# CV-Project2025/Project-NeRF

Measured on NVIDIA B200. Metric: train_rays_per_s, higher is better.
Workload: dtype f16

## Files before the change

### include/b2nerf.h

```cpp
#ifndef B2NERF_H_
#define B2NERF_H_

#include <stddef.h>
#include <stdint.h>

#ifdef __cplusplus
extern "C" {
#endif

#define B2N_ABI_VERSION 14

#define B2N_OK 0
#define B2N_EINVAL (-1)
#define B2N_ECUDA (-2)

typedef void* b2n_stream_t;

int b2n_abi_version(void);
const char* b2n_last_error(void);

int b2n_set_active_rows(const int* rows_device);

enum { B2N_ACT_NONE = 0, B2N_ACT_RELU = 1, B2N_ACT_SIGMOID = 2 };


int b2n_occ_pack_bits(const uint8_t* binary, int64_t n_voxels, uint32_t* bits, b2n_stream_t stream);

int b2n_occ_active_mask(const float* pts, int64_t P, const uint32_t* bits, int R, float offset, float scale,
                        uint8_t* mask, b2n_stream_t stream);

int b2n_occ_update(const float* cur_sigma, float* grid, int64_t n_voxels, int dynamic, float decay, float threshold,
                   uint8_t* binary, uint32_t* bits, int64_t* n_active, b2n_stream_t stream);

int b2n_march_mask(const float* rays_o, const float* rays_d, const float* z_base, const float* z_lo,
                   const float* z_hi, const float* u, const uint32_t* bits, int R, float offset, float scale,
                   int64_t B, int N, float* z, uint32_t* mask_words, int32_t* ray_count, b2n_stream_t stream);

size_t b2n_march_scan_scratch(int64_t B);
int b2n_march_scan(int32_t* ray_count, uint32_t* mask_words, int W, int64_t B, int32_t* ray_offset,
                   int32_t* total_out, void* scratch, b2n_stream_t stream);

int b2n_march_compact(const float* rays_o, const float* rays_d, const float* times, const float* z,
                      const uint32_t* mask_words, const int32_t* ray_offset, int64_t B, int N,
                      int32_t* sample_idx, float* pts, float* dirs, float* t_out, b2n_stream_t stream);

int b2n_composite_fwd(const float* rgb, const float* sigma, const float* dx, const float* z, const float* rays_d,
                      const float* bg, int bg_per_ray, const uint32_t* mask_words, const int32_t* ray_offset,
                      int64_t B, int N, float* color, float* depth, float* acc, float* mean_dx,
                      b2n_stream_t stream);
int b2n_composite_bwd(const float* rgb, const float* sigma, const float* dx, const float* z, const float* rays_d,
                      const float* bg, int bg_per_ray, const uint32_t* mask_words, const int32_t* ray_offset,
                      int64_t B, int N, const float* g_color, const float* g_depth, const float* g_acc,
                      const float* g_mean_dx, float* g_rgb, float* g_sigma, float* g_dx, b2n_stream_t stream);

int b2n_pe_fwd(const float* x, int64_t P, int D, const float* bands, int L, float* out, int ld_out, int col0,
               b2n_stream_t stream);
int b2n_pe_bwd(const float* x, int64_t P, int D, const float* bands, int L, const float* g_out, int ld_g, int col0,
               float* g_x, int accumulate, b2n_stream_t stream);

#define B2N_MAX_LEVELS 32
typedef struct {
  float scale;
  uint32_t res;
  uint32_t size;
  uint32_t offset;
  uint32_t hashed;
} b2n_hash_level;

int b2n_hash_fwd(const float* x, int64_t P, float bound, const float* table, const b2n_hash_level* levels_host,
                 int L, int F, float* out, int ld_out, int col0, b2n_stream_t stream);
int b2n_hash_bwd(const float* x, int64_t P, float bound, const float* table, const b2n_hash_level* levels_host,
                 int L, int F, const float* g_out, int ld_g, int col0, float* g_table, float* g_x, int accumulate_x,
                 int level_begin, int level_end, b2n_stream_t stream);

int b2n_hash_tri_fwd(const float* x, const float* t, int64_t P, float bound, const float* table_start,
                     const float* table_mid, const float* table_end, const b2n_hash_level* levels_host, int L,
                     float* out, int ld_out, b2n_stream_t stream);
int b2n_hash_tri_bwd(const float* x, const float* t, int64_t P, float bound, const b2n_hash_level* levels_host, int L,
                     const float* g_out, int ld_g, float* g_table_start, float* g_table_mid, float* g_table_end,
                     b2n_stream_t stream);

int b2n_linear_fwd(const float* X, int ldx, const float* W, int ldw, const float* b, float* Y, int ldy, int64_t P,
                   int K, int N, int act, b2n_stream_t stream);
int b2n_linear_dgrad(const float* dY, int lddy, const float* W, int ldw, const float* Xact, int ldxa, int act,
                     float* dX, int lddx, int64_t P, int K, int N, int accumulate, b2n_stream_t stream);
int b2n_linear_wgrad(const float* dY, int lddy, const float* X, int ldx, float* dW, int lddw, float* db, int64_t P,
                     int K, int N, b2n_stream_t stream);
int b2n_act_bwd(float* dY, int lddy, const float* Y, int ldy, int64_t P, int N, int act, b2n_stream_t stream);

int b2n_sigma_head_fwd(const float* h, int ldh, int64_t P, float* sigma, b2n_stream_t stream);
int b2n_sigma_head_bwd(const float* h, int ldh, int64_t P, const float* g_sigma, float* g_h, int ldg,
                       b2n_stream_t stream);

int b2n_instant_mlp_fwd(const float* x_enc, int ldx, int pos_dim, const float* dirs, const float* dir_bands,
                        int L_dir, const float* sigma_params, const float* color_params, int64_t P, float* rgb,
                        float* sigma, float in_pad_value, b2n_stream_t stream);
int b2n_instant_mlp_fwd_tc(const float* x_enc, int ldx, int pos_dim, const float* dirs, const float* dir_bands,
                           int L_dir, const float* sigma_params, const float* color_params, int64_t P, float* rgb,
                           float* sigma, float in_pad_value, int* err_flag, b2n_stream_t stream);
int b2n_instant_mlp_bwd(const float* x_enc, int ldx, int pos_dim, const float* dirs, const float* dir_bands,
                        int L_dir, const float* sigma_params, const float* color_params, int64_t P,
                        const float* g_rgb, const float* g_sigma, float* g_x_enc, int ldg, float* g_sigma_params,
                        float* g_color_params, void* work4, float in_pad_value, b2n_stream_t stream);
int b2n_instant_mlp_bwd_tc(const float* x_enc, int ldx, int pos_dim, const float* dirs, const float* dir_bands,
                           int L_dir, const float* sigma_params, const float* color_params, int64_t P,
                           const float* g_rgb, const float* g_sigma, float* g_x_enc, int ldg, float* g_sigma_params,
// ... 65 lines not shown
```

### project-nerf_b200/b2n/_lib.py

```python
from __future__ import annotations

import ctypes
import os

import torch

_HERE = os.path.dirname(os.path.abspath(__file__))
LIB_PATH = os.path.join(os.path.dirname(_HERE), "lib", "libb2nerf.so")

ABI_VERSION = 14

P, L, I, F = ctypes.c_void_p, ctypes.c_int64, ctypes.c_int, ctypes.c_float

SIGNATURES = {
    "b2n_abi_version": [],
    "b2n_last_error": [],
    "b2n_set_active_rows": [P],
    "b2n_occ_pack_bits": [P, L, P, P],
    "b2n_occ_active_mask": [P, L, P, I, F, F, P, P],
    "b2n_occ_update": [P, P, L, I, F, F, P, P, P, P],
    "b2n_march_mask": [P, P, P, P, P, P, P, I, F, F, L, I, P, P, P, P],
    "b2n_march_scan_scratch": [L],
    "b2n_march_scan": [P, P, I, L, P, P, P, P],
    "b2n_march_compact": [P, P, P, P, P, P, L, I, P, P, P, P, P],
    "b2n_composite_fwd": [P, P, P, P, P, P, I, P, P, L, I, P, P, P, P, P],
    "b2n_composite_bwd": [P, P, P, P, P, P, I, P, P, L, I, P, P, P, P, P, P, P, P],
    "b2n_pe_fwd": [P, L, I, P, I, P, I, I, P],
    "b2n_pe_bwd": [P, L, I, P, I, P, I, I, P, I, P],
    "b2n_hash_fwd": [P, L, F, P, P, I, I, P, I, I, P],
    "b2n_hash_bwd": [P, L, F, P, P, I, I, P, I, I, P, P, I, I, I, P],
    "b2n_hash_tri_fwd": [P, P, L, F, P, P, P, P, I, P, I, P],
    "b2n_hash_tri_bwd": [P, P, L, F, P, I, P, I, P, P, P, P],
    "b2n_linear_fwd": [P, I, P, I, P, P, I, L, I, I, I, P],
    "b2n_linear_dgrad": [P, I, P, I, P, I, I, P, I, L, I, I, I, P],
    "b2n_linear_wgrad": [P, I, P, I, P, I, P, L, I, I, P],
    "b2n_act_bwd": [P, I, P, I, L, I, I, P],
    "b2n_sigma_head_fwd": [P, I, L, P, P],
    "b2n_sigma_head_bwd": [P, I, L, P, P, I, P],
    "b2n_instant_mlp_fwd": [P, I, I, P, P, I, P, P, L, P, P, F, P],
    "b2n_instant_mlp_fwd_tc": [P, I, I, P, P, I, P, P, L, P, P, F, P, P],
    "b2n_instant_mlp_bwd": [P, I, I, P, P, I, P, P, L, P, P, P, I, P, P, P, F, P],
    "b2n_instant_mlp_bwd_tc": [P, I, I, P, P, I, P, P, L, P, P, P, I, P, P, P, F, P, P],
    "b2n_fmlp_in_pad": [I],
    "b2n_fmlp_out_pad": [I],
    "b2n_fmlp_fwd": [P, I, I, P, I, I, I, I, P, P, P, I, I, L, P, I, P, P, P],
    "b2n_fmlp_bwd": [I, I, I, I, P, P, I, I, L, P, I, P, I, P, P, P, P, I, P, I, P, P],
    "b2n_fmlp_wgrad_tc": [P, P, P, P, L, I, I, I, P, P, P, P, P, P, P],
    "b2n_fmlp_wgrad": [I, P, P, P, P, P, P, P, P, P, P, P, L, P, P],
    "b2n_nerf_mlp_wgrad": [P, P, P, I, P, L, P, P, P, P, P, P, P, P],
    "b2n_nerf_mlp_dx": [P, P, P, I, P, I, I, L, P, I, P],
    "b2n_nerf_mlp_head_wgrad": [P, P, P, L, P, P, P, P],
    "b2n_nerf_mlp_packed_bytes": [],
    "b2n_nerf_mlp_pack": [P, P, P, I, I, P, P],
    "b2n_nerf_mlp_fwd": [P, I, P, I, P, P, P, P, P, L, P, P, P, P, P, P],
    "b2n_pad_bf16": [P, L, I, I, P, P],
    "b2n_opt_prepare": [P, I, P, P, P],
    "b2n_opt_adamw": [P, I, P, I, P, P, P, P, P],
    "b2n_sample_rays": [P, P, P, P, P, P, L, I, I, I, F, F, P, P, P, P, P],
    "b2n_nerf_mlp_packed_bwd_bytes": [],
    "b2n_nerf_mlp_pack_bwd": [P, P, P, I, I, P, P],
    "b2n_nerf_mlp_bwd": [P, P, P, P, P, P, P, P, L, P, P, P, P],
}
DEBUG_SIGNATURES = {
    "b2n_debug_mlp256_prof": [P],
    "b2n_debug_mlp256_flags": [ctypes.c_int],
    "b2n_debug_mlp256_set_pair": [ctypes.c_int],
    "b2n_debug_hash_variant": [I, I],
    "b2n_debug_hash_config": [P, P],
    "b2n_debug_instant_bwd_groups": [I],
    "b2n_debug_instant_fwd_slots": [I],
    "b2n_debug_gather_bench": [P, L, I, I, P, P],
    "b2n_debug_red_bench": [P, L, I, I, I, P],
    "b2n_debug_mnmajor_probe": [P, P, P, I, I, I, I, P],
}
_RESTYPES = {"b2n_last_error": ctypes.c_char_p, "b2n_march_scan_scratch": ctypes.c_size_t,
             "b2n_nerf_mlp_packed_bytes": ctypes.c_size_t, "b2n_nerf_mlp_packed_bwd_bytes": ctypes.c_size_t}


class HashLevelC(ctypes.Structure):
    _fields_ = [("scale", ctypes.c_float), ("res", ctypes.c_uint32), ("size", ctypes.c_uint32),
                ("offset", ctypes.c_uint32), ("hashed", ctypes.c_uint32)]


def _load():
    if not os.path.exists(LIB_PATH):
        raise ImportError(
            f"{LIB_PATH} not found: build the CUDA extension first (python project-nerf_b200/build.py). "
            "This package has no CPU fallback.")
    lib = ctypes.CDLL(LIB_PATH)
    for name, argtypes in list(SIGNATURES.items()) + list(DEBUG_SIGNATURES.items()):
        fn = getattr(lib, name)
        fn.argtypes = argtypes
        fn.restype = _RESTYPES.get(name, ctypes.c_int)
    v = lib.b2n_abi_version()
    if v != ABI_VERSION:
        raise ImportError(f"libb2nerf.so ABI {v} != binding ABI {ABI_VERSION}: rebuild")
    return lib


lib = _load()

LAUNCHES = {"count": 0}
_KERNELS_PER_CALL = {"b2n_march_scan": 3, "b2n_linear_wgrad": 2, "b2n_instant_mlp_bwd": 2, "b2n_instant_mlp_bwd_tc": 2, "b2n_fmlp_bwd": 2}


def ptr(t):
    return None if t is None else t.data_ptr()


def stream():
    return torch.cuda.current_stream().cuda_stream


class Profiler:

    def __init__(self):
        self.records = []

    def summary(self):
        out = {}
        for name, nbytes, flops, e0, e1 in self.records:
            d = out.setdefault(name, dict(calls=0, ms=0.0, bytes=0.0, flops=0.0))
            d["calls"] += 1
            d["ms"] += e0.elapsed_time(e1)
            d["bytes"] += nbytes
            d["flops"] += flops
        return out


PROFILER = None


def call(name: str, *args, work=(0.0, 0.0)):
    prof = PROFILER
    if prof is not None:
        e0 = torch.cuda.Event(enable_timing=True)
        e1 = torch.cuda.Event(enable_timing=True)
        e0.record()
    rc = getattr(lib, name)(*args)
    if prof is not None:
        e1.record()
        prof.records.append((name, float(work[0]), float(work[1]), e0, e1))
    _raise_on(name, rc)
    LAUNCHES["count"] += _KERNELS_PER_CALL.get(name, 1)


def _raise_on(name, rc):
    if rc != 0:
        msg = lib.b2n_last_error().decode(errors="replace")
        if rc == -1:
            raise ValueError(f"{name}: {msg}")
        raise RuntimeError(f"{name} failed ({rc}): {msg}")


def hash_config():
    v, m = ctypes.c_int(), ctypes.c_int()
    _raise_on("b2n_debug_hash_config", lib.b2n_debug_hash_config(ctypes.byref(v), ctypes.byref(m)))
    return v.value, m.value


class hash_variant:

    def __init__(self, variant, merge_res):
        self.cfg = (variant, merge_res)

    def __enter__(self):
        self.prev = hash_config()
        _raise_on("b2n_debug_hash_variant", lib.b2n_debug_hash_variant(*self.cfg))
        return self

    def __exit__(self, *exc):
        _raise_on("b2n_debug_hash_variant", lib.b2n_debug_hash_variant(*self.prev))
        return False


# ... 53 lines not shown
```

### project-nerf_b200/b2n/ops.py

```python
from __future__ import annotations

import ctypes
import math
from typing import List, Optional, Sequence

import numpy as np
import torch
from torch.amp import custom_bwd, custom_fwd

from . import _lib
from ._lib import HashLevelC, current_rows, ptr, require_cuda, stream, with_ctx_rows

import os as _os
INSTANT_FWD_TC = _os.environ.get("B2N_INSTANT_TC", "1") != "0"
INSTANT_BWD_TC = _os.environ.get("B2N_INSTANT_BWD_TC", "1") != "0"


def call(name, *args, work=(0.0, 0.0)):
    _lib.call(name, *args, work=work)

ACT_NONE, ACT_RELU, ACT_SIGMOID = 0, 1, 2
_ACT = {"none": ACT_NONE, "relu": ACT_RELU, "sigmoid": ACT_SIGMOID}


def _narrow_out(*shape, device, dtype=torch.float32):
    if current_rows() is not None:
        return torch.zeros(*shape, device=device, dtype=dtype)
    return torch.empty(*shape, device=device, dtype=dtype)


def _c(t: Optional[torch.Tensor]) -> Optional[torch.Tensor]:
    if t is None:
        return None
    if t.dtype != torch.float32:
        t = t.float()
    return t.contiguous()



_libm = ctypes.CDLL("libm.so.6")
for _fn in ("exp2f", "log2f", "ceilf"):
    getattr(_libm, _fn).restype = ctypes.c_float
    getattr(_libm, _fn).argtypes = [ctypes.c_float]


class HashGeometry:

    def __init__(self, n_levels: int, base_resolution: int, per_level_scale: float, log2_hashmap_size: int,
# ... 6 lines not shown
        log2s = _libm.log2f(ctypes.c_float(per_level_scale))
        arr = (HashLevelC * n_levels)()
        offset = 0
        self.levels = []
        for l in range(n_levels):
            e = float(np.float32(np.float32(l) * np.float32(log2s)))
            scale = np.float32(np.float32(_libm.exp2f(ctypes.c_float(e))) * np.float32(base_resolution)) - np.float32(1.0)
            res = int(_libm.ceilf(ctypes.c_float(float(scale)))) + 1
            dense = res ** 3
            size = min((min(dense, (1 << 31) - 1) + 7) // 8 * 8, 1 << log2_hashmap_size)
            hashed = size < dense
            arr[l] = HashLevelC(float(scale), res, size, offset, int(hashed))
            self.levels.append((float(scale), res, size, offset, hashed))
            offset += size
        self.c_levels = arr
        self.n_entries = offset
        self.n_params = offset * n_features
        self.out_dim = n_levels * n_features


class _HashEncode(torch.autograd.Function):
    @staticmethod
    @custom_fwd(device_type="cuda", cast_inputs=torch.float32)
    def forward(ctx, x, table, geom: HashGeometry, bound: float, sink):
        require_cuda(x, table)
        ctx.rows = current_rows()
        x, table = _c(x), _c(table)
        if x.dim() != 2 or x.shape[1] != 3:
            raise ValueError("hash_encode expects x of shape [P, 3]")
        if table.numel() != geom.n_params:
            raise ValueError(f"hash table has {table.numel()} params, geometry needs {geom.n_params}")
        Pn = x.shape[0]
        out = torch.empty(Pn, geom.out_dim, device=x.device, dtype=torch.float32)
        call("b2n_hash_fwd", ptr(x), Pn, float(bound), ptr(table), geom.c_levels, geom.n_levels, geom.n_features,
             ptr(out), geom.out_dim, 0, stream(),
             work=(Pn * (12 + geom.n_levels * geom.n_features * 4 * 9), 0.0))
        ctx.save_for_backward(x, table)
        ctx.geom, ctx.bound = geom, bound
        ctx.sink = sink if (sink is not None and ctx.needs_input_grad[1]) else None
        if ctx.sink is not None:
            ctx.sink.uses += 1
        return out

    @staticmethod
    @custom_bwd(device_type="cuda")
    @with_ctx_rows
    def backward(ctx, g):
        x, table = ctx.saved_tensors
        geom = ctx.geom
        g = _c(g)
        need_x, need_t = ctx.needs_input_grad[0], ctx.needs_input_grad[1]
        g_x = torch.empty_like(x) if need_x else None
        Pn, L, F = x.shape[0], geom.n_levels, geom.n_features
        bytes_t = (12 + L * F * 4 * 17) * int(need_t)
        bytes_x = (24 + L * F * 4 * 9) * int(need_x)

        def launch(g_table, gx, lo, hi, nbytes):
            call("b2n_hash_bwd", ptr(x), Pn, float(ctx.bound), ptr(table), geom.c_levels, L, F, ptr(g), geom.out_dim, 0,
                 ptr(g_table), ptr(gx), 0, lo, hi, stream(), work=(Pn * nbytes, 0.0))

        sink = ctx.sink
        if sink is None or not need_t:
            g_table = torch.zeros_like(table) if need_t else None
            if need_x or need_t:
                launch(g_table, g_x, 0, -1, bytes_t + bytes_x)
            return g_x, g_table, None, None, None
        sink.uses -= 1
        last = sink.uses <= 0
        split = sink.split_level if (last and F == 2 and 0 < sink.split_level < L and sink.split_level % 4 == 0) else 0
        if split:
            cut = geom.levels[split][3] * F
            launch(sink.view, None, split, L, bytes_t * (L - split) / L)
            sink.on_ready(sink, cut, sink.view.numel())
            launch(sink.view, g_x, 0, split, bytes_t * split / L + bytes_x)
            sink.on_ready(sink, 0, cut)
        else:
            launch(sink.view, g_x, 0, -1, bytes_t + bytes_x)
            if last:
                sink.on_ready(sink, 0, sink.view.numel())
        return g_x, None, None, None, None


def hash_encode(x, table, geom: HashGeometry, bound: float):
    sink = getattr(table, "_b2n_grad_sink", None) if torch.is_grad_enabled() else None
    return _HashEncode.apply(x, table, geom, bound, sink)


class _HashTriBlend(torch.autograd.Function):

    @staticmethod
# ... 623 lines not shown
```

### project-nerf_b200/csrc/b2n_encode.cu

```cuda
#include "b2n_common.cuh"
#include "b2n_hash.cuh"

namespace b2n {

#define B2N_PI_F 3.14159274101257324f

__global__ void __launch_bounds__(256) k_pe_fwd(const float* __restrict__ x, int64_t P, int D, const float* __restrict__ bands,
                                                int L, float* __restrict__ out, int ld, int col0, const int* __restrict__ rows) {
  P = clamp_rows(P, rows);
  const int slots = L + 1, pts = 256 / slots;
  const int lp = threadIdx.x / slots, k = threadIdx.x - lp * slots;
  const int64_t p = (int64_t)blockIdx.x * pts + lp;
  if (lp >= pts || p >= P) return;
  const float* xp = x + p * D;
  float* row = out + p * ld + col0;
  if (k == 0) {
    for (int d = 0; d < D; ++d) row[d] = xp[d];
  } else {
    const float f = __ldg(bands + k - 1);
    float* dst = row + D + 2 * (k - 1) * D;
    for (int d = 0; d < D; ++d) {
      const float arg = __fmul_rn(__fmul_rn(xp[d], f), B2N_PI_F);
      float sn, cs;
      sincosf(arg, &sn, &cs);
      dst[d] = sn;
      dst[D + d] = cs;
    }
  }
}

__global__ void k_pe_bwd(const float* __restrict__ x, int64_t P, int D, const float* __restrict__ bands, int L,
                         const float* __restrict__ g, int ld, int col0, float* __restrict__ gx, int accumulate, const int* __restrict__ rows) {
  P = clamp_rows(P, rows);
  int64_t i = (int64_t)blockIdx.x * blockDim.x + threadIdx.x;
// ... 194 lines not shown
      for (int s = 0; s < steps; ++s) {
        const int o = 1 << s;
        float t[F];
#pragma unroll
        for (int f = 0; f < F; ++f) t[f] = __shfl_down_sync(0xffffffffu, v[f], o);
        const bool same_run = (lane + o < 32) && (((heads >> (lane + 1)) & ((1u << o) - 1u)) == 0u);
        if (same_run) {
#pragma unroll
          for (int f = 0; f < F; ++f) v[f] += t[f];
        }
      }
      if (issuer) {
        const uint32_t e = corner_entry(L, c.g[0] + (k & 1), c.g[1] + ((k >> 1) & 1), c.g[2] + ((k >> 2) & 1));
        bool any = false;
#pragma unroll
        for (int f = 0; f < F; ++f) any |= (v[f] != 0.f);
        if (any) {
          if (F == 2) {
            atomicAdd(reinterpret_cast<float2*>(g_table) + e, make_float2(v[0], v[1]));
          } else if (F == 4) {
            atomicAdd(reinterpret_cast<float4*>(g_table) + e, make_float4(v[0], v[1], v[2], v[3]));
          } else {
#pragma unroll
            for (int f = 0; f < F; ++f) atomicAdd(g_table + (size_t)e * F + f, v[f]);
          }
        }
      }
    }
  }
}

__device__ __forceinline__ float pair_sum(float v) { return v + __shfl_xor_sync(0xffffffffu, v, 1); }

__global__ void __launch_bounds__(256)
k_hash_fwd_pair(const float* __restrict__ x, int64_t P, float bound, float two_bound, const float2* __restrict__ table,
                const Levels lv, int nl, float* __restrict__ out, int ld, int col0, const int* __restrict__ rows) {
  P = clamp_rows(P, rows);
  if ((int64_t)blockIdx.x * (blockDim.x >> 1) >= P) return;
  const int64_t tid = (int64_t)blockIdx.x * blockDim.x + threadIdx.x;
  const int64_t p = tid >> 1;
  const int s = threadIdx.x & 1;
  const bool live = p < P;
  float x01[3] = {0.f, 0.f, 0.f};
  if (live) {
    bool in;
#pragma unroll
    for (int d = 0; d < 3; ++d) x01[d] = to_unit(__ldg(x + 3 * p + d), bound, two_bound, &in);
  }
  float* orow = out + p * ld + col0;
  const bool vec = ((reinterpret_cast<uintptr_t>(out + col0) & 15) == 0) && ((ld & 3) == 0);
  __shared__ float4 stage[8][16 * 10];
  const bool contig = vec && col0 == 0 && ld == 2 * nl && ld <= 32 && (nl & 1) == 0 &&
                      (uint64_t)(lv.l[nl - 1].offset + lv.l[nl - 1].size) * 8u <= (64ull << 20);
  const int warp = threadIdx.x >> 5, lane = threadIdx.x & 31, pi = lane >> 1;
  for (int l0 = 0; l0 < nl; l0 += 4) {
    float keep0 = 0.f, keep1 = 0.f, keep2 = 0.f, keep3 = 0.f;
#pragma unroll
    for (int j = 0; j < 4; ++j) {
      const int l = l0 + j;
      float a0 = 0.f, a1 = 0.f;
      if (l < nl) {
        const b2n_hash_level L = lv.l[l];
        const Cell c = locate(x01, L.scale);
        const uint32_t cx = c.g[0] + (uint32_t)s;
        const float wx = s ? c.w[0] : 1.f - c.w[0];
        float2 v[4];
#pragma unroll
        for (int k = 0; k < 4; ++k) {
          const uint32_t e = corner_entry(L, cx, c.g[1] + (k & 1), c.g[2] + (k >> 1));
          v[k] = live ? __ldg(table + e) : make_float2(0.f, 0.f);
        }
#pragma unroll
        for (int k = 0; k < 4; ++k) {
          const float w = wx * ((k & 1) ? c.w[1] : 1.f - c.w[1]) * ((k & 2) ? c.w[2] : 1.f - c.w[2]);
          a0 += w * v[k].x, a1 += w * v[k].y;
        }
      }
      a0 = pair_sum(a0), a1 = pair_sum(a1);
      if ((j >> 1) == s) {
        if (j & 1) keep2 = a0, keep3 = a1;
        else keep0 = a0, keep1 = a1;
      }
    }
    const int lf = l0 + 2 * s;
    if (contig) {
      if (lf + 1 < nl) stage[warp][pi * 10 + (lf >> 1)] = make_float4(keep0, keep1, keep2, keep3);
    } else if (live) {
      float* o = orow + 2 * lf;
      if (vec && lf + 1 < nl) {
        __stcs(reinterpret_cast<float4*>(o), make_float4(keep0, keep1, keep2, keep3));
      } else {
        if (lf < nl) __stcs(o, keep0), __stcs(o + 1, keep1);
        if (lf + 1 < nl) __stcs(o + 2, keep2), __stcs(o + 3, keep3);
      }
    }
  }
  if (contig) {
    __syncwarp();
    const int64_t p_warp = ((int64_t)blockIdx.x * blockDim.x + 32 * warp) >> 1;
    const int per_row = ld >> 2;
    const int n4 = 16 * per_row;
    float4* dst = reinterpret_cast<float4*>(out + p_warp * ld);
    for (int i = lane; i < n4; i += 32) {
      const int row = i / per_row, col = i - row * per_row;
      if (p_warp + row < P) __stcs(dst + i, stage[warp][row * 10 + col]);
    }
  }
}

__global__ void __launch_bounds__(256)
k_hash_bwd_table_pair(const float* __restrict__ x, int64_t P, float bound, float two_bound, const Levels lv, int lbeg,
                      int nl, const float* __restrict__ g, int ld, int col0, float2* __restrict__ g_table,
                      uint32_t merge_res, const int* __restrict__ rows) {
  P = clamp_rows(P, rows);
  if ((int64_t)blockIdx.x * (blockDim.x >> 1) >= P) return;
  const int64_t tid = (int64_t)blockIdx.x * blockDim.x + threadIdx.x;
  const int64_t p = tid >> 1;
  const int lane = threadIdx.x & 31, s = lane & 1, pi = lane >> 1;
  const bool live = p < P;
  float x01[3] = {0.f, 0.f, 0.f};
  if (live) {
    bool in;
#pragma unroll
    for (int d = 0; d < 3; ++d) x01[d] = to_unit(__ldg(x + 3 * p + d), bound, two_bound, &in);
  }
  const float* grow = g + p * ld + col0;
  const bool vec = ((reinterpret_cast<uintptr_t>(g + col0) & 15) == 0) && ((ld & 3) == 0);
  for (int l0 = lbeg; l0 < nl; l0 += 4) {
    float gv[8] = {0.f, 0.f, 0.f, 0.f, 0.f, 0.f, 0.f, 0.f};
    if (live) {
      if (vec && l0 + 4 <= nl) {
        const float4 a = __ldcs(reinterpret_cast<const float4*>(grow + 2 * l0));
        const float4 b = __ldcs(reinterpret_cast<const float4*>(grow + 2 * l0) + 1);
        gv[0] = a.x, gv[1] = a.y, gv[2] = a.z, gv[3] = a.w, gv[4] = b.x, gv[5] = b.y, gv[6] = b.z, gv[7] = b.w;
      } else {
#pragma unroll
        for (int j = 0; j < 8; ++j)
          if (2 * l0 + j < 2 * nl) gv[j] = __ldcs(grow + 2 * l0 + j);
      }
    }
#pragma unroll
    for (int j = 0; j < 4; ++j) {
      const int l = l0 + j;
      if (l >= nl) break;
      const b2n_hash_level L = lv.l[l];
      const Cell c = locate(x01, L.scale);
      const uint32_t cx = c.g[0] + (uint32_t)s;
      const float wx = s ? c.w[0] : 1.f - c.w[0];
      const float g0 = gv[2 * j], g1 = gv[2 * j + 1];
      if (L.res > merge_res) {
        if (live && (g0 != 0.f || g1 != 0.f)) {
#pragma unroll
          for (int k = 0; k < 4; ++k) {
            const float w = wx * ((k & 1) ? c.w[1] : 1.f - c.w[1]) * ((k & 2) ? c.w[2] : 1.f - c.w[2]);
            atomicAdd(g_table + corner_entry(L, cx, c.g[1] + (k & 1), c.g[2] + (k >> 1)), make_float2(w * g0, w * g1));
          }
        }
        continue;
      }
      const uint32_t cell = live ? (c.g[0] + c.g[1] * L.res + c.g[2] * L.res * L.res) : (0xffffffffu - (uint32_t)pi);
      const uint32_t cell_prev = __shfl_up_sync(0xffffffffu, cell, 2);
      const bool head = (pi == 0) || (cell != cell_prev);
      const uint32_t heads = __ballot_sync(0xffffffffu, head && s == 0);
      const int steps = L.res <= 24 ? 3 : (L.res <= 64 ? 2 : 1);
      const int run_start = (31 - __clz((int)(heads & (0xffffffffu >> (31 - 2 * pi))))) >> 1;
      const bool issuer = live && (((pi - run_start) & ((1 << steps) - 1)) == 0);
#pragma unroll
      for (int k = 0; k < 4; ++k) {
        const float w = wx * ((k & 1) ? c.w[1] : 1.f - c.w[1]) * ((k & 2) ? c.w[2] : 1.f - c.w[2]);
        float v0 = w * g0, v1 = w * g1;
        for (int st = 0; st < steps; ++st) {
          const int o = 1 << st;
          const float t0 = __shfl_down_sync(0xffffffffu, v0, 2 * o), t1 = __shfl_down_sync(0xffffffffu, v1, 2 * o);
          const uint32_t span = (o == 1) ? 0x1u : (o == 2 ? 0x5u : 0x55u);
          const bool same_run = (pi + o < 16) && (((heads >> (2 * (pi + 1))) & span) == 0u);
          if (same_run) v0 += t0, v1 += t1;
        }
        if (issuer && (v0 != 0.f || v1 != 0.f))
          atomicAdd(g_table + corner_entry(L, cx, c.g[1] + (k & 1), c.g[2] + (k >> 1)), make_float2(v0, v1));
      }
    }
  }
}

template <int F>
__global__ void __launch_bounds__(256)
k_hash_bwd_input(const float* __restrict__ x, int64_t P, float bound, float two_bound,
                 const float* __restrict__ table, const Levels lv, int nl, const float* __restrict__ g, int ld,
                 int col0, float* __restrict__ gx, int accumulate, const int* __restrict__ rows) {
  P = clamp_rows(P, rows);
  const int64_t p = (int64_t)blockIdx.x * blockDim.x + threadIdx.x;
  if (p >= P) return;
  bool in[3];
  float x01[3];
#pragma unroll
  for (int d = 0; d < 3; ++d) x01[d] = to_unit(__ldg(x + 3 * p + d), bound, two_bound, &in[d]);
  float gsum[3] = {0.f, 0.f, 0.f};
  const float* gi = g + p * ld + col0;
  for (int l = 0; l < nl; ++l) {
    const b2n_hash_level L = lv.l[l];
    const Cell c = locate(x01, L.scale);
    float gv[F];
#pragma unroll
    for (int f = 0; f < F; ++f) gv[f] = gi[l * F + f];
    float dot[8];
#pragma unroll
    for (int k = 0; k < 8; ++k) {
// ... 190 lines not shown
    if (h[i].hashed && (h[i].size & (h[i].size - 1))) return -1;
  }
  return 0;
}

}

using namespace b2n;

extern "C" int b2n_pe_fwd(const float* x, int64_t P, int D, const float* bands, int L, float* out, int ld_out,
                          int col0, b2n_stream_t stream) {
  B2N_REQUIRE(P >= 0 && D > 0 && D <= 4 && L >= 0 && L <= 32, "bad shape");
  if (P == 0) return B2N_OK;
  B2N_REQUIRE(x && out && (L == 0 || bands), "null pointer");
  B2N_REQUIRE(ld_out >= col0 + D + 2 * D * L && col0 >= 0, "output row too narrow");
  const int pts_per_block = 256 / (L + 1);
  const int64_t blocks = (P + pts_per_block - 1) / pts_per_block;
  B2N_REQUIRE(blocks <= 0x7fffffffLL, "too many points for one launch");
  k_pe_fwd<<<(unsigned)blocks, 256, 0, (cudaStream_t)stream>>>(x, P, D, bands, L, out, ld_out, col0, g_active_rows);
  return check_launch("b2n_pe_fwd");
}

extern "C" int b2n_pe_bwd(const float* x, int64_t P, int D, const float* bands, int L, const float* g_out, int ld_g,
                          int col0, float* g_x, int accumulate, b2n_stream_t stream) {
  B2N_REQUIRE(P >= 0 && D > 0 && D <= 4 && L >= 0 && L <= 32, "bad shape");
  if (P == 0) return B2N_OK;
  B2N_REQUIRE(x && g_out && g_x && (L == 0 || bands), "null pointer");
  B2N_REQUIRE(ld_g >= col0 + D + 2 * D * L && col0 >= 0, "gradient row too narrow");
  k_pe_bwd<<<grid_for(P * D, 256), 256, 0, (cudaStream_t)stream>>>(x, P, D, bands, L, g_out, ld_g, col0, g_x,
                                                                  accumulate, g_active_rows);
  return check_launch("b2n_pe_bwd");
}

extern "C" int b2n_hash_fwd(const float* x, int64_t P, float bound, const float* table,
                            const b2n_hash_level* levels_host, int L, int F, float* out, int ld_out, int col0,
                            b2n_stream_t stream) {
  B2N_REQUIRE(P >= 0 && (F == 1 || F == 2 || F == 4) && bound >= 0.f, "bad shape (F in {1,2,4})");
  Levels lv;
  B2N_REQUIRE(fill_levels(levels_host, L, &lv) == 0, "bad level table");
  if (P == 0) return B2N_OK;
  B2N_REQUIRE(x && table && out, "null pointer");
  B2N_REQUIRE((reinterpret_cast<uintptr_t>(table) & 15) == 0, "table must be 16-byte aligned (vector gathers)");
  B2N_REQUIRE(ld_out >= col0 + L * F && col0 >= 0, "output row too narrow");
  const unsigned grid = grid_for(P * L, 256);
  const float tb = 2.0f * bound;
  cudaStream_t st = (cudaStream_t)stream;
  if (F == 2 && (g_hash_variant & 1))
    k_hash_fwd_pair<<<grid_for(2 * P, 256), 256, 0, st>>>(x, P, bound, tb, reinterpret_cast<const float2*>(table), lv, L, out,
                                                        ld_out, col0, g_active_rows);
  else if (F == 2) k_hash_fwd<2><<<grid, 256, 0, st>>>(x, P, bound, tb, table, lv, L, out, ld_out, col0, g_active_rows);
  else if (F == 4) k_hash_fwd<4><<<grid, 256, 0, st>>>(x, P, bound, tb, table, lv, L, out, ld_out, col0, g_active_rows);
  else k_hash_fwd<1><<<grid, 256, 0, st>>>(x, P, bound, tb, table, lv, L, out, ld_out, col0, g_active_rows);
  return check_launch("b2n_hash_fwd");
}

extern "C" int b2n_hash_bwd(const float* x, int64_t P, float bound, const float* table,
                            const b2n_hash_level* levels_host, int L, int F, const float* g_out, int ld_g, int col0,
                            float* g_table, float* g_x, int accumulate_x, int level_begin, int level_end,
                            b2n_stream_t stream) {
  B2N_REQUIRE(P >= 0 && (F == 1 || F == 2 || F == 4) && bound >= 0.f, "bad shape (F in {1,2,4})");
  if (level_end < 0) level_end = L;
  B2N_REQUIRE(level_begin >= 0 && level_begin <= level_end && level_end <= L, "bad level window");
  const bool windowed = level_begin != 0 || level_end != L;
  B2N_REQUIRE(!windowed || (F == 2 && (level_begin & 3) == 0), "a level window needs F = 2 and a start that is a multiple of 4");
  Levels lv;
  B2N_REQUIRE(fill_levels(levels_host, L, &lv) == 0, "bad level table");
  if (P == 0) return B2N_OK;
  B2N_REQUIRE(x && g_out, "null pointer");
  B2N_REQUIRE(ld_g >= col0 + L * F && col0 >= 0, "gradient row too narrow");
  B2N_REQUIRE(!g_x || table, "input gradient needs the table");
  B2N_REQUIRE((reinterpret_cast<uintptr_t>(g_table) & 15) == 0 && (reinterpret_cast<uintptr_t>(table) & 15) == 0,
              "table / g_table must be 16-byte aligned (vector reductions)");
  const float tb = 2.0f * bound;
  cudaStream_t st = (cudaStream_t)stream;
  if (g_table && F == 2 && ((g_hash_variant & 2) || windowed)) {
    if (level_begin < level_end)
      k_hash_bwd_table_pair<<<grid_for(2 * P, 256), 256, 0, st>>>(x, P, bound, tb, lv, level_begin, level_end, g_out, ld_g,
                                                                col0, reinterpret_cast<float2*>(g_table), g_merge_res, g_active_rows);
  } else if (g_table) {
    int n_dense = 0;
    while (n_dense < L && !lv.l[n_dense].hashed) ++n_dense;
    if (n_dense > 0) {
      const unsigned gd = grid_for(P, 256);
      if (F == 2) k_hash_bwd_table_dense<2><<<gd, 256, 0, st>>>(x, P, bound, tb, lv, n_dense, g_out, ld_g, col0, g_table, g_active_rows);
      else if (F == 4) k_hash_bwd_table_dense<4><<<gd, 256, 0, st>>>(x, P, bound, tb, lv, n_dense, g_out, ld_g, col0, g_table, g_active_rows);
      else k_hash_bwd_table_dense<1><<<gd, 256, 0, st>>>(x, P, bound, tb, lv, n_dense, g_out, ld_g, col0, g_table, g_active_rows);
    }
    if (n_dense < L) {
      const unsigned grid = grid_for(P * (L - n_dense), 256);
      if (F == 2) k_hash_bwd_table<2><<<grid, 256, 0, st>>>(x, P, bound, tb, lv, L, n_dense, g_out, ld_g, col0, g_table, g_active_rows);
      else if (F == 4) k_hash_bwd_table<4><<<grid, 256, 0, st>>>(x, P, bound, tb, lv, L, n_dense, g_out, ld_g, col0, g_table, g_active_rows);
      else k_hash_bwd_table<1><<<grid, 256, 0, st>>>(x, P, bound, tb, lv, L, n_dense, g_out, ld_g, col0, g_table, g_active_rows);
    }
  }
  if (g_x) {
    const unsigned grid = grid_for(P, 256);
    if (F == 2 && (g_hash_variant & 1))
      k_hash_bwd_input_pair<<<grid_for(2 * P, 256), 256, 0, st>>>(x, P, bound, tb, reinterpret_cast<const float2*>(table), lv, L, g_out,
                                                                ld_g, col0, g_x, accumulate_x, g_active_rows);
    else if (F == 2) k_hash_bwd_input<2><<<grid, 256, 0, st>>>(x, P, bound, tb, table, lv, L, g_out, ld_g, col0, g_x, accumulate_x, g_active_rows);
    else if (F == 4) k_hash_bwd_input<4><<<grid, 256, 0, st>>>(x, P, bound, tb, table, lv, L, g_out, ld_g, col0, g_x, accumulate_x, g_active_rows);
    else k_hash_bwd_input<1><<<grid, 256, 0, st>>>(x, P, bound, tb, table, lv, L, g_out, ld_g, col0, g_x, accumulate_x, g_active_rows);
  }
  return check_launch("b2n_hash_bwd");
}

extern "C" int b2n_hash_tri_fwd(const float* x, const float* t, int64_t P, float bound, const float* table_start,
                                const float* table_mid, const float* table_end, const b2n_hash_level* levels_host, int L,
                                float* out, int ld_out, b2n_stream_t stream) {
  B2N_REQUIRE(P >= 0 && bound >= 0.f, "bad shape");
  Levels lv;
  B2N_REQUIRE(fill_levels(levels_host, L, &lv) == 0, "bad level table");
  if (P == 0) return B2N_OK;
  B2N_REQUIRE(x && t && table_start && table_mid && table_end && out, "null pointer");
  B2N_REQUIRE(ld_out >= 2 * L && (ld_out & 1) == 0 && (reinterpret_cast<uintptr_t>(out) & 7) == 0, "output row too narrow / unaligned");
  const TriTables tabs{{table_start, table_mid, table_end}};
  k_hash_tri_fwd<<<grid_for(P * L, 256), 256, 0, (cudaStream_t)stream>>>(x, t, P, bound, 2.0f * bound, tabs, lv, L, out, ld_out, g_active_rows);
  return check_launch("b2n_hash_tri_fwd");
}

extern "C" int b2n_hash_tri_bwd(const float* x, const float* t, int64_t P, float bound, const b2n_hash_level* levels_host,
                                int L, const float* g_out, int ld_g, float* g_table_start, float* g_table_mid,
                                float* g_table_end, b2n_stream_t stream) {
  B2N_REQUIRE(P >= 0 && bound >= 0.f, "bad shape");
  Levels lv;
  B2N_REQUIRE(fill_levels(levels_host, L, &lv) == 0, "bad level table");
  if (P == 0) return B2N_OK;
  B2N_REQUIRE(x && t && g_out, "null pointer");
  B2N_REQUIRE(ld_g >= 2 * L && (ld_g & 1) == 0 && (reinterpret_cast<uintptr_t>(g_out) & 7) == 0, "gradient row too narrow / unaligned");
  const TriGrads grads{{g_table_start, g_table_mid, g_table_end}};
  k_hash_tri_bwd<<<grid_for(P * L, 256), 256, 0, (cudaStream_t)stream>>>(x, t, P, bound, 2.0f * bound, lv, L, g_out, ld_g, grads, g_active_rows);
  return check_launch("b2n_hash_tri_bwd");
}

extern "C" int b2n_debug_hash_variant(int variant, int merge_res) {
  B2N_REQUIRE(variant >= 0 && variant <= 3, "variant must be in 0..3");
  B2N_REQUIRE(merge_res <= 1625, "merge_res must be <= 1625 (1626^3 overflows the uint32 cell id)");
// ... 12 lines not shown
```

Measured before the change: 12.27 million.

## Sort hash-encoding points by Morton key for locality in forward and backward

Adds a counting-sort pass that groups sample points by a 21-bit Morton key over a 128^3 grid. It writes a permutation and a sorted copy of the coordinates, and new ordered hash forward and backward kernels read the sorted points and scatter outputs and gradients through the permutation. Block order is also interleaved across a spread of blocks so that concurrently running blocks touch different spatial regions, and the backward widens its run-merging steps because sorted warps hold more repeated cells. The goal is better cache locality for table gathers and fewer atomic reductions, at the cost of five extra kernels plus a memset, scattered output writes, and extra memory. It only runs for at least 2^23 points with F=2, no input gradient, and hash config variant 3.

```diff
diff --git a/include/b2nerf.h b/include/b2nerf.h
--- a/include/b2nerf.h
+++ b/include/b2nerf.h
@@ -8,7 +8,7 @@
 extern "C" {
 #endif
 
-#define B2N_ABI_VERSION 14
+#define B2N_ABI_VERSION 15
 
 #define B2N_OK 0
 #define B2N_EINVAL (-1)
@@ -72,6 +72,16 @@
 int b2n_hash_bwd(const float* x, int64_t P, float bound, const float* table, const b2n_hash_level* levels_host,
                  int L, int F, const float* g_out, int ld_g, int col0, float* g_table, float* g_x, int accumulate_x,
                  int level_begin, int level_end, b2n_stream_t stream);
+
+size_t b2n_hash_order_scratch(int64_t P);
+int b2n_hash_order(const float* x, int64_t P, float bound, int* order, float* x_sorted, void* scratch,
+                   b2n_stream_t stream);
+int b2n_hash_fwd_ordered(const float* x_sorted, const int* order, int64_t P, float bound, const float* table,
+                         const b2n_hash_level* levels_host, int L, int F, float* out, int ld_out, int col0,
+                         b2n_stream_t stream);
+int b2n_hash_bwd_ordered(const float* x_sorted, const int* order, int64_t P, float bound, const float* table,
+                         const b2n_hash_level* levels_host, int L, int F, const float* g_out, int ld_g, int col0,
+                         float* g_table, int level_begin, int level_end, b2n_stream_t stream);
 
 int b2n_hash_tri_fwd(const float* x, const float* t, int64_t P, float bound, const float* table_start,
                      const float* table_mid, const float* table_end, const b2n_hash_level* levels_host, int L,
diff --git a/project-nerf_b200/b2n/_lib.py b/project-nerf_b200/b2n/_lib.py
--- a/project-nerf_b200/b2n/_lib.py
+++ b/project-nerf_b200/b2n/_lib.py
@@ -8,7 +8,7 @@
 _HERE = os.path.dirname(os.path.abspath(__file__))
 LIB_PATH = os.path.join(os.path.dirname(_HERE), "lib", "libb2nerf.so")
 
-ABI_VERSION = 14
+ABI_VERSION = 15
 
 P, L, I, F = ctypes.c_void_p, ctypes.c_int64, ctypes.c_int, ctypes.c_float
 
@@ -29,6 +29,10 @@
     "b2n_pe_bwd": [P, L, I, P, I, P, I, I, P, I, P],
     "b2n_hash_fwd": [P, L, F, P, P, I, I, P, I, I, P],
     "b2n_hash_bwd": [P, L, F, P, P, I, I, P, I, I, P, P, I, I, I, P],
+    "b2n_hash_order_scratch": [L],
+    "b2n_hash_order": [P, L, F, P, P, P, P],
+    "b2n_hash_fwd_ordered": [P, P, L, F, P, P, I, I, P, I, I, P],
+    "b2n_hash_bwd_ordered": [P, P, L, F, P, P, I, I, P, I, I, P, I, I, P],
     "b2n_hash_tri_fwd": [P, P, L, F, P, P, P, P, I, P, I, P],
     "b2n_hash_tri_bwd": [P, P, L, F, P, I, P, I, P, P, P, P],
     "b2n_linear_fwd": [P, I, P, I, P, P, I, L, I, I, I, P],
@@ -73,7 +77,7 @@
     "b2n_debug_red_bench": [P, L, I, I, I, P],
     "b2n_debug_mnmajor_probe": [P, P, P, I, I, I, I, P],
 }
-_RESTYPES = {"b2n_last_error": ctypes.c_char_p, "b2n_march_scan_scratch": ctypes.c_size_t,
+_RESTYPES = {"b2n_last_error": ctypes.c_char_p, "b2n_march_scan_scratch": ctypes.c_size_t, "b2n_hash_order_scratch": ctypes.c_size_t,
              "b2n_nerf_mlp_packed_bytes": ctypes.c_size_t, "b2n_nerf_mlp_packed_bwd_bytes": ctypes.c_size_t}
 
 
@@ -101,7 +105,7 @@
 lib = _load()
 
 LAUNCHES = {"count": 0}
-_KERNELS_PER_CALL = {"b2n_march_scan": 3, "b2n_linear_wgrad": 2, "b2n_instant_mlp_bwd": 2, "b2n_instant_mlp_bwd_tc": 2, "b2n_fmlp_bwd": 2}
+_KERNELS_PER_CALL = {"b2n_march_scan": 3, "b2n_hash_order": 5, "b2n_linear_wgrad": 2, "b2n_instant_mlp_bwd": 2, "b2n_instant_mlp_bwd_tc": 2, "b2n_fmlp_bwd": 2}
 
 
 def ptr(t):
@@ -129,6 +133,7 @@
 
 
 PROFILER = None
+_PROFILE_AS = {"b2n_hash_fwd_ordered": "b2n_hash_fwd", "b2n_hash_bwd_ordered": "b2n_hash_bwd"}
 
 
 def call(name: str, *args, work=(0.0, 0.0)):
@@ -140,7 +145,7 @@
     rc = getattr(lib, name)(*args)
     if prof is not None:
         e1.record()
-        prof.records.append((name, float(work[0]), float(work[1]), e0, e1))
+        prof.records.append((_PROFILE_AS.get(name, name), float(work[0]), float(work[1]), e0, e1))
     _raise_on(name, rc)
     LAUNCHES["count"] += _KERNELS_PER_CALL.get(name, 1)
 
diff --git a/project-nerf_b200/b2n/ops.py b/project-nerf_b200/b2n/ops.py
--- a/project-nerf_b200/b2n/ops.py
+++ b/project-nerf_b200/b2n/ops.py
@@ -14,6 +14,7 @@
 import os as _os
 INSTANT_FWD_TC = _os.environ.get("B2N_INSTANT_TC", "1") != "0"
 INSTANT_BWD_TC = _os.environ.get("B2N_INSTANT_BWD_TC", "1") != "0"
+HASH_ORDER_MIN_POINTS = 1 << 23
 
 
 def call(name, *args, work=(0.0, 0.0)):
@@ -86,9 +87,20 @@
             raise ValueError(f"hash table has {table.numel()} params, geometry needs {geom.n_params}")
         Pn = x.shape[0]
         out = torch.empty(Pn, geom.out_dim, device=x.device, dtype=torch.float32)
-        call("b2n_hash_fwd", ptr(x), Pn, float(bound), ptr(table), geom.c_levels, geom.n_levels, geom.n_features,
-             ptr(out), geom.out_dim, 0, stream(),
-             work=(Pn * (12 + geom.n_levels * geom.n_features * 4 * 9), 0.0))
+        work = (Pn * (12 + geom.n_levels * geom.n_features * 4 * 9), 0.0)
+        ctx.order = None
+        if Pn >= HASH_ORDER_MIN_POINTS and geom.n_features == 2 and not ctx.needs_input_grad[0] and _lib.hash_config()[0] == 3:
+            order = torch.empty(Pn, device=x.device, dtype=torch.int32)
+            xs = torch.empty_like(x)
+            scratch = torch.empty(_lib.lib.b2n_hash_order_scratch(Pn) // 4, device=x.device, dtype=torch.int32)
+            call("b2n_hash_order", ptr(x), Pn, float(bound), ptr(order), ptr(xs), ptr(scratch), stream(),
+                 work=(Pn * (12 + 4 + 4 + 12 + 4 + 12), 0.0))
+            call("b2n_hash_fwd_ordered", ptr(xs), ptr(order), Pn, float(bound), ptr(table), geom.c_levels, geom.n_levels,
+                 geom.n_features, ptr(out), geom.out_dim, 0, stream(), work=work)
+            x, ctx.order = xs, order
+        else:
+            call("b2n_hash_fwd", ptr(x), Pn, float(bound), ptr(table), geom.c_levels, geom.n_levels, geom.n_features,
+                 ptr(out), geom.out_dim, 0, stream(), work=work)
         ctx.save_for_backward(x, table)
         ctx.geom, ctx.bound = geom, bound
         ctx.sink = sink if (sink is not None and ctx.needs_input_grad[1]) else None
@@ -110,6 +122,10 @@
         bytes_x = (24 + L * F * 4 * 9) * int(need_x)
 
         def launch(g_table, gx, lo, hi, nbytes):
+            if ctx.order is not None:
+                call("b2n_hash_bwd_ordered", ptr(x), ptr(ctx.order), Pn, float(ctx.bound), ptr(table), geom.c_levels, L,
+                     F, ptr(g), geom.out_dim, 0, ptr(g_table), lo, hi, stream(), work=(Pn * nbytes, 0.0))
+                return
             call("b2n_hash_bwd", ptr(x), Pn, float(ctx.bound), ptr(table), geom.c_levels, L, F, ptr(g), geom.out_dim, 0,
                  ptr(g_table), ptr(gx), 0, lo, hi, stream(), work=(Pn * nbytes, 0.0))
 
diff --git a/project-nerf_b200/csrc/b2n_encode.cu b/project-nerf_b200/csrc/b2n_encode.cu
--- a/project-nerf_b200/csrc/b2n_encode.cu
+++ b/project-nerf_b200/csrc/b2n_encode.cu
@@ -1,5 +1,6 @@
 #include "b2n_common.cuh"
 #include "b2n_hash.cuh"
+#include <cub/block/block_scan.cuh>
 
 namespace b2n {
 
@@ -260,13 +261,108 @@
 
 __device__ __forceinline__ float pair_sum(float v) { return v + __shfl_xor_sync(0xffffffffu, v, 1); }
 
+constexpr int kOrderBits = 7;
+constexpr int kOrderBuckets = 1 << (3 * kOrderBits);
+constexpr int kOrderTile = 2048;
+constexpr int kOrderTiles = kOrderBuckets / kOrderTile;
+constexpr int kSpread = 2048;
+
+__device__ __forceinline__ uint32_t spread3(uint32_t v) {
+  v = (v | (v << 16)) & 0x030000FFu;
+  v = (v | (v << 8)) & 0x0300F00Fu;
+  v = (v | (v << 4)) & 0x030C30C3u;
+  return (v | (v << 2)) & 0x09249249u;
+}
+
+__device__ __forceinline__ uint32_t order_key(const float* __restrict__ x, int64_t p, float bound, float two_bound) {
+  uint32_t q[3];
+#pragma unroll
+  for (int d = 0; d < 3; ++d) {
+    bool in;
+    const float u = to_unit(__ldg(x + 3 * p + d), bound, two_bound, &in);
+    q[d] = min((uint32_t)(u * (float)(1 << kOrderBits)), (uint32_t)((1 << kOrderBits) - 1));
+  }
+  return spread3(q[0]) | (spread3(q[1]) << 1) | (spread3(q[2]) << 2);
+}
+
+__device__ __forceinline__ int64_t block_first_point(int64_t P, bool ordered) {
+  if (!ordered) return (int64_t)blockIdx.x * 128;
+  const int64_t nc = (P + 127) / 128, R = (nc + kSpread - 1) / kSpread, b = blockIdx.x;
+  if (b / kSpread >= R) return -1;
+  const int64_t c = (b % kSpread) * R + b / kSpread;
+  return c < nc ? c * 128 : -1;
+}
+
+__global__ void __launch_bounds__(256)
+k_order_count(const float* __restrict__ x, int64_t P, float bound, float two_bound, int* __restrict__ counts,
+              int* __restrict__ rank, const int* __restrict__ rows) {
+  P = clamp_rows(P, rows);
+  const int64_t p = (int64_t)blockIdx.x * blockDim.x + threadIdx.x;
+  if (p < P) rank[p] = atomicAdd(counts + order_key(x, p, bound, two_bound), 1);
+}
+
+__global__ void __launch_bounds__(256) k_order_scan_tiles(int* __restrict__ counts, int* __restrict__ tile_sum) {
+  using Scan = cub::BlockScan<int, 256>;
+  __shared__ typename Scan::TempStorage tmp;
+  int4* base = reinterpret_cast<int4*>(counts + (int64_t)blockIdx.x * kOrderTile) + 2 * threadIdx.x;
+  const int4 a = base[0], b = base[1];
+  int v[8] = {a.x, a.y, a.z, a.w, b.x, b.y, b.z, b.w};
+  int tot = 0;
+#pragma unroll
+  for (int i = 0; i < 8; ++i) tot += v[i];
+  int pre, all;
+  Scan(tmp).ExclusiveSum(tot, pre, all);
+#pragma unroll
+  for (int i = 0; i < 8; ++i) {
+    const int t = v[i];
+    v[i] = pre;
+    pre += t;
+  }
+  base[0] = make_int4(v[0], v[1], v[2], v[3]);
+  base[1] = make_int4(v[4], v[5], v[6], v[7]);
+  if (threadIdx.x == 0) tile_sum[blockIdx.x] = all;
+}
+
+__global__ void __launch_bounds__(kOrderTiles) k_order_scan_top(int* __restrict__ tile_sum) {
+  using Scan = cub::BlockScan<int, kOrderTiles>;
+  __shared__ typename Scan::TempStorage tmp;
+  int v = tile_sum[threadIdx.x];
+  Scan(tmp).ExclusiveSum(v, v);
+  tile_sum[threadIdx.x] = v;
+}
+
+__global__ void __launch_bounds__(256)
+k_order_scatter(const float* __restrict__ x, int64_t P_cap, float bound, float two_bound, const int* __restrict__ counts,
+                const int* __restrict__ tile_sum, const int* __restrict__ rank, int* __restrict__ order,
+                const int* __restrict__ rows) {
+  const int64_t P = clamp_rows(P_cap, rows);
+  const int64_t p = (int64_t)blockIdx.x * blockDim.x + threadIdx.x;
+  if (p >= P_cap) return;
+  int64_t pos = p;
+  if (p < P) {
+    const uint32_t k = order_key(x, p, bound, two_bound);
+    pos = (int64_t)__ldg(tile_sum + k / kOrderTile) + __ldg(counts + k) + rank[p];
+  }
+  order[pos] = (int)p;
+}
+
+__global__ void __launch_bounds__(256)
+k_order_gather(const float* __restrict__ x, int64_t P_cap, const int* __restrict__ order, float* __restrict__ xs) {
+  const int64_t i = (int64_t)blockIdx.x * blockDim.x + threadIdx.x;
+  if (i >= P_cap) return;
+  const int64_t p = __ldg(order + i);
+#pragma unroll
+  for (int d = 0; d < 3; ++d) xs[3 * i + d] = __ldg(x + 3 * p + d);
+}
+
 __global__ void __launch_bounds__(256)
 k_hash_fwd_pair(const float* __restrict__ x, int64_t P, float bound, float two_bound, const float2* __restrict__ table,
-                const Levels lv, int nl, float* __restrict__ out, int ld, int col0, const int* __restrict__ rows) {
-  P = clamp_rows(P, rows);
-  if ((int64_t)blockIdx.x * (blockDim.x >> 1) >= P) return;
-  const int64_t tid = (int64_t)blockIdx.x * blockDim.x + threadIdx.x;
-  const int64_t p = tid >> 1;
+                const Levels lv, int nl, float* __restrict__ out, int ld, int col0, const int* __restrict__ order,
+                const int* __restrict__ rows) {
+  P = clamp_rows(P, rows);
+  const int64_t p_block = block_first_point(P, order != nullptr);
+  if (p_block < 0 || p_block >= P) return;
+  const int64_t p = p_block + (threadIdx.x >> 1);
   const int s = threadIdx.x & 1;
   const bool live = p < P;
   float x01[3] = {0.f, 0.f, 0.f};
@@ -275,7 +371,7 @@
 #pragma unroll
     for (int d = 0; d < 3; ++d) x01[d] = to_unit(__ldg(x + 3 * p + d), bound, two_bound, &in);
   }
-  float* orow = out + p * ld + col0;
+  float* orow = out + (order && live ? (int64_t)__ldg(order + p) : p) * ld + col0;
   const bool vec = ((reinterpret_cast<uintptr_t>(out + col0) & 15) == 0) && ((ld & 3) == 0);
   __shared__ float4 stage[8][16 * 10];
   const bool contig = vec && col0 == 0 && ld == 2 * nl && ld <= 32 && (nl & 1) == 0 &&
@@ -325,13 +421,14 @@
   }
   if (contig) {
     __syncwarp();
-    const int64_t p_warp = ((int64_t)blockIdx.x * blockDim.x + 32 * warp) >> 1;
+    const int64_t p_warp = p_block + 16 * warp;
     const int per_row = ld >> 2;
     const int n4 = 16 * per_row;
-    float4* dst = reinterpret_cast<float4*>(out + p_warp * ld);
     for (int i = lane; i < n4; i += 32) {
       const int row = i / per_row, col = i - row * per_row;
-      if (p_warp + row < P) __stcs(dst + i, stage[warp][row * 10 + col]);
+      const int64_t pr = p_warp + row;
+      if (pr < P) __stcs(reinterpret_cast<float4*>(out + (order ? (int64_t)__ldg(order + pr) : pr) * ld) + col,
+                         stage[warp][row * 10 + col]);
     }
   }
 }
@@ -339,11 +436,11 @@
 __global__ void __launch_bounds__(256)
 k_hash_bwd_table_pair(const float* __restrict__ x, int64_t P, float bound, float two_bound, const Levels lv, int lbeg,
                       int nl, const float* __restrict__ g, int ld, int col0, float2* __restrict__ g_table,
-                      uint32_t merge_res, const int* __restrict__ rows) {
-  P = clamp_rows(P, rows);
-  if ((int64_t)blockIdx.x * (blockDim.x >> 1) >= P) return;
-  const int64_t tid = (int64_t)blockIdx.x * blockDim.x + threadIdx.x;
-  const int64_t p = tid >> 1;
+                      uint32_t merge_res, const int* __restrict__ order, const int* __restrict__ rows) {
+  P = clamp_rows(P, rows);
+  const int64_t p_block = block_first_point(P, order != nullptr);
+  if (p_block < 0 || p_block >= P) return;
+  const int64_t p = p_block + (threadIdx.x >> 1);
   const int lane = threadIdx.x & 31, s = lane & 1, pi = lane >> 1;
   const bool live = p < P;
   float x01[3] = {0.f, 0.f, 0.f};
@@ -352,7 +449,7 @@
 #pragma unroll
     for (int d = 0; d < 3; ++d) x01[d] = to_unit(__ldg(x + 3 * p + d), bound, two_bound, &in);
   }
-  const float* grow = g + p * ld + col0;
+  const float* grow = g + (order && live ? (int64_t)__ldg(order + p) : p) * ld + col0;
   const bool vec = ((reinterpret_cast<uintptr_t>(g + col0) & 15) == 0) && ((ld & 3) == 0);
   for (int l0 = lbeg; l0 < nl; l0 += 4) {
     float gv[8] = {0.f, 0.f, 0.f, 0.f, 0.f, 0.f, 0.f, 0.f};
@@ -390,7 +487,7 @@
       const uint32_t cell_prev = __shfl_up_sync(0xffffffffu, cell, 2);
       const bool head = (pi == 0) || (cell != cell_prev);
       const uint32_t heads = __ballot_sync(0xffffffffu, head && s == 0);
-      const int steps = L.res <= 24 ? 3 : (L.res <= 64 ? 2 : 1);
+      const int steps = order ? (L.res <= 54 ? 4 : (L.res <= 122 ? 3 : 2)) : (L.res <= 24 ? 3 : (L.res <= 64 ? 2 : 1));
       const int run_start = (31 - __clz((int)(heads & (0xffffffffu >> (31 - 2 * pi))))) >> 1;
       const bool issuer = live && (((pi - run_start) & ((1 << steps) - 1)) == 0);
 #pragma unroll
@@ -400,7 +497,7 @@
         for (int st = 0; st < steps; ++st) {
           const int o = 1 << st;
           const float t0 = __shfl_down_sync(0xffffffffu, v0, 2 * o), t1 = __shfl_down_sync(0xffffffffu, v1, 2 * o);
-          const uint32_t span = (o == 1) ? 0x1u : (o == 2 ? 0x5u : 0x55u);
+          const uint32_t span = ((1u << (2 * o)) - 1u) & 0x55555555u;
           const bool same_run = (pi + o < 16) && (((heads >> (2 * (pi + 1))) & span) == 0u);
           if (same_run) v0 += t0, v1 += t1;
         }
@@ -657,10 +754,15 @@
   return check_launch("b2n_pe_bwd");
 }
 
-extern "C" int b2n_hash_fwd(const float* x, int64_t P, float bound, const float* table,
-                            const b2n_hash_level* levels_host, int L, int F, float* out, int ld_out, int col0,
-                            b2n_stream_t stream) {
+static unsigned pair_grid(int64_t P, const int* order) {
+  const int64_t g = (P + 127) / 128;
+  return (unsigned)(order ? (g + kSpread - 1) / kSpread * kSpread : (g < 1 ? 1 : g));
+}
+
+static int hash_fwd(const float* x, const int* order, int64_t P, float bound, const float* table,
+                    const b2n_hash_level* levels_host, int L, int F, float* out, int ld_out, int col0, b2n_stream_t stream) {
   B2N_REQUIRE(P >= 0 && (F == 1 || F == 2 || F == 4) && bound >= 0.f, "bad shape (F in {1,2,4})");
+  B2N_REQUIRE(!order || (F == 2 && (g_hash_variant & 1)), "an order needs F = 2 and the pair-lane forward");
   Levels lv;
   B2N_REQUIRE(fill_levels(levels_host, L, &lv) == 0, "bad level table");
   if (P == 0) return B2N_OK;
@@ -671,18 +773,17 @@
   const float tb = 2.0f * bound;
   cudaStream_t st = (cudaStream_t)stream;
   if (F == 2 && (g_hash_variant & 1))
-    k_hash_fwd_pair<<<grid_for(2 * P, 256), 256, 0, st>>>(x, P, bound, tb, reinterpret_cast<const float2*>(table), lv, L, out,
-                                                        ld_out, col0, g_active_rows);
+    k_hash_fwd_pair<<<pair_grid(P, order), 256, 0, st>>>(x, P, bound, tb, reinterpret_cast<const float2*>(table), lv, L, out,
+                                                       ld_out, col0, order, g_active_rows);
   else if (F == 2) k_hash_fwd<2><<<grid, 256, 0, st>>>(x, P, bound, tb, table, lv, L, out, ld_out, col0, g_active_rows);
   else if (F == 4) k_hash_fwd<4><<<grid, 256, 0, st>>>(x, P, bound, tb, table, lv, L, out, ld_out, col0, g_active_rows);
   else k_hash_fwd<1><<<grid, 256, 0, st>>>(x, P, bound, tb, table, lv, L, out, ld_out, col0, g_active_rows);
   return check_launch("b2n_hash_fwd");
 }
 
-extern "C" int b2n_hash_bwd(const float* x, int64_t P, float bound, const float* table,
-                            const b2n_hash_level* levels_host, int L, int F, const float* g_out, int ld_g, int col0,
-                            float* g_table, float* g_x, int accumulate_x, int level_begin, int level_end,
-                            b2n_stream_t stream) {
+static int hash_bwd(const float* x, const int* order, int64_t P, float bound, const float* table,
+                    const b2n_hash_level* levels_host, int L, int F, const float* g_out, int ld_g, int col0,
+                    float* g_table, float* g_x, int accumulate_x, int level_begin, int level_end, b2n_stream_t stream) {
   B2N_REQUIRE(P >= 0 && (F == 1 || F == 2 || F == 4) && bound >= 0.f, "bad shape (F in {1,2,4})");
   if (level_end < 0) level_end = L;
   B2N_REQUIRE(level_begin >= 0 && level_begin <= level_end && level_end <= L, "bad level window");
@@ -696,12 +797,15 @@
   B2N_REQUIRE(!g_x || table, "input gradient needs the table");
   B2N_REQUIRE((reinterpret_cast<uintptr_t>(g_table) & 15) == 0 && (reinterpret_cast<uintptr_t>(table) & 15) == 0,
               "table / g_table must be 16-byte aligned (vector reductions)");
+  B2N_REQUIRE(!order || (!g_x && F == 2 && ((g_hash_variant & 2) || windowed)),
+              "an order needs F = 2, the pair-lane table gradient and no input gradient");
   const float tb = 2.0f * bound;
   cudaStream_t st = (cudaStream_t)stream;
   if (g_table && F == 2 && ((g_hash_variant & 2) || windowed)) {
     if (level_begin < level_end)
-      k_hash_bwd_table_pair<<<grid_for(2 * P, 256), 256, 0, st>>>(x, P, bound, tb, lv, level_begin, level_end, g_out, ld_g,
-                                                                col0, reinterpret_cast<float2*>(g_table), g_merge_res, g_active_rows);
+      k_hash_bwd_table_pair<<<pair_grid(P, order), 256, 0, st>>>(x, P, bound, tb, lv, level_begin, level_end, g_out, ld_g,
+                                                               col0, reinterpret_cast<float2*>(g_table), g_merge_res, order,
+                                                               g_active_rows);
   } else if (g_table) {
     int n_dense = 0;
     while (n_dense < L && !lv.l[n_dense].hashed) ++n_dense;
@@ -728,6 +832,59 @@
     else k_hash_bwd_input<1><<<grid, 256, 0, st>>>(x, P, bound, tb, table, lv, L, g_out, ld_g, col0, g_x, accumulate_x, g_active_rows);
   }
   return check_launch("b2n_hash_bwd");
+}
+
+extern "C" int b2n_hash_fwd(const float* x, int64_t P, float bound, const float* table,
+                            const b2n_hash_level* levels_host, int L, int F, float* out, int ld_out, int col0,
+                            b2n_stream_t stream) {
+  return hash_fwd(x, nullptr, P, bound, table, levels_host, L, F, out, ld_out, col0, stream);
+}
+
+extern "C" int b2n_hash_fwd_ordered(const float* x_sorted, const int* order, int64_t P, float bound, const float* table,
+                                    const b2n_hash_level* levels_host, int L, int F, float* out, int ld_out, int col0,
+                                    b2n_stream_t stream) {
+  B2N_REQUIRE(order, "null order");
+  return hash_fwd(x_sorted, order, P, bound, table, levels_host, L, F, out, ld_out, col0, stream);
+}
+
+extern "C" int b2n_hash_bwd(const float* x, int64_t P, float bound, const float* table,
+                            const b2n_hash_level* levels_host, int L, int F, const float* g_out, int ld_g, int col0,
+                            float* g_table, float* g_x, int accumulate_x, int level_begin, int level_end,
+                            b2n_stream_t stream) {
+  return hash_bwd(x, nullptr, P, bound, table, levels_host, L, F, g_out, ld_g, col0, g_table, g_x, accumulate_x,
+                  level_begin, level_end, stream);
+}
+
+extern "C" int b2n_hash_bwd_ordered(const float* x_sorted, const int* order, int64_t P, float bound, const float* table,
+                                    const b2n_hash_level* levels_host, int L, int F, const float* g_out, int ld_g,
+                                    int col0, float* g_table, int level_begin, int level_end, b2n_stream_t stream) {
+  B2N_REQUIRE(order, "null order");
+  return hash_bwd(x_sorted, order, P, bound, table, levels_host, L, F, g_out, ld_g, col0, g_table, nullptr, 0,
+                  level_begin, level_end, stream);
+}
+
+extern "C" size_t b2n_hash_order_scratch(int64_t P) {
+  return sizeof(int) * ((size_t)kOrderBuckets + kOrderTiles + (size_t)(P > 0 ? P : 0));
+}
+
+extern "C" int b2n_hash_order(const float* x, int64_t P, float bound, int* order, float* x_sorted, void* scratch,
+                              b2n_stream_t stream) {
+  B2N_REQUIRE(P >= 0 && P < (1LL << 31) && bound >= 0.f, "bad shape (P < 2^31 rows)");
+  if (P == 0) return B2N_OK;
+  B2N_REQUIRE(x && order && x_sorted && scratch, "null pointer");
+  B2N_REQUIRE((reinterpret_cast<uintptr_t>(scratch) & 15) == 0, "scratch must be 16-byte aligned");
+  int* counts = static_cast<int*>(scratch);
+  int* tile_sum = counts + kOrderBuckets;
+  int* rank = tile_sum + kOrderTiles;
+  cudaStream_t st = (cudaStream_t)stream;
+  const float tb = 2.0f * bound;
+  if (cudaMemsetAsync(counts, 0, sizeof(int) * kOrderBuckets, st) != cudaSuccess) return check_launch("b2n_hash_order");
+  k_order_count<<<grid_for(P, 256), 256, 0, st>>>(x, P, bound, tb, counts, rank, g_active_rows);
+  k_order_scan_tiles<<<kOrderTiles, 256, 0, st>>>(counts, tile_sum);
+  k_order_scan_top<<<1, kOrderTiles, 0, st>>>(tile_sum);
+  k_order_scatter<<<grid_for(P, 256), 256, 0, st>>>(x, P, bound, tb, counts, tile_sum, rank, order, g_active_rows);
+  k_order_gather<<<grid_for(P, 256), 256, 0, st>>>(x, P, order, x_sorted);
+  return check_launch("b2n_hash_order");
 }
 
 extern "C" int b2n_hash_tri_fwd(const float* x, const float* t, int64_t P, float bound, const float* table_start,
```

New measurement: 12.86 million, median of 6. +4.9%, better.
